# nickgreenquist/cu2rec

Measured on AMD Instinct MI355X. Metric: ratings/sec (SGD updates/sec), higher is better.
Workload: dtype f32

## Files before the change

cu2rec_amd/csrc/blocksolve.hip:

```cpp
#include <hip/hip_runtime.h>
#include <hip/hip_ext.h>

#include <algorithm>
#include <atomic>
#include <cmath>
#include <cstdlib>
#include <limits>
#include <mutex>
#include <string>
#include <utility>
#include <vector>

#include "blocksolve.hpp"
#include "blocksolve_device.hpp"
#include "blocksolve_gram.hpp"
#include "blocksolve_lookahead.hpp"
#include "blocksolve_solve.hpp"
#include "blocksolve_update.hpp"
#include "hip_check.hpp"

namespace cu2rec {

namespace {

using namespace bs_dev;

__global__ void bs_tables_kernel(SgdHyper h, float *__restrict__ t) {
    const int k = threadIdx.x;
    if (k > 2 * kB) return;
    const double a = 1.0 - static_cast<double>(h.lr) * static_cast<double>(h.q_reg);
    const double c = 1.0 - static_cast<double>(h.lr) * static_cast<double>(h.ib_reg);
    double ak = 1.0, ck = 1.0;
    for (int i = 0; i < k; ++i) {
        ak *= a;
        ck *= c;
    }
    t[kTabAdel + k] = static_cast<float>(1.0 - ak);
    t[kTabCdel + k] = static_cast<float>(1.0 - ck);
    t[kTabApow + k] = static_cast<float>(ak);
    t[kTabCpow + k] = static_cast<float>(ck);
}

__device__ __forceinline__ int lower_bound_key(const uint32_t *__restrict__ keys, int n, uint32_t target) {
    int lo = 0, hi = n;
    while (lo < hi) {
        const int mid = (lo + hi) >> 1;
        if (keys[mid] < target) lo = mid + 1; else hi = mid;
    }
    return lo;
}

__global__ __launch_bounds__(256) void bs_plan_kernel(const uint32_t *__restrict__ keys, int n_active, int n_hot,
                                                      int item_bits, int max_blocks, const int *__restrict__ item_of_rank,
                                                      int *__restrict__ chain_begin, BsChainDesc *__restrict__ chains,
                                                      BsBlockDesc *__restrict__ blocks, int *__restrict__ walk_begin, size_t stride) {
    __shared__ int s_part[256];
    const int b = blockIdx.x, tid = threadIdx.x;
    const uint32_t *kb = keys + static_cast<size_t>(b) * stride;
    int *cb = chain_begin + static_cast<size_t>(b) * (n_hot + 1);
    BsChainDesc *cd = chains + static_cast<size_t>(b) * max(n_hot, 1);
    BsBlockDesc *bd = blocks + static_cast<size_t>(b) * max_blocks;
    for (int r = tid; r <= n_hot; r += 256) cb[r] = lower_bound_key(kb, n_active, static_cast<uint32_t>(r));
    __syncthreads();
    if (tid == 0) walk_begin[b] = cb[n_hot];
    const int per = (n_hot + 255) / 256;
    const int r0 = min(tid * per, n_hot), r1 = min(r0 + per, n_hot);
    int mine = 0;
    for (int r = r0; r < r1; ++r) mine += (cb[r + 1] - cb[r] + kB - 1) / kB;
    s_part[tid] = mine;
    __syncthreads();
    __shared__ int s_total;
    if (tid == 0) {
        int run = 0;
        for (int t = 0; t < 256; ++t) {
            const int v = s_part[t];
            s_part[t] = run;
            run += v;
        }
        s_total = run;
    }
    __syncthreads();
    int off = s_part[tid];
    for (int r = r0; r < r1; ++r) {
        const int begin = cb[r], len = cb[r + 1] - begin;
        cd[r] = BsChainDesc{begin, len, off, item_of_rank[r]};
        const int nb = (len + kB - 1) / kB;
        for (int m = 0; m < nb; ++m) bd[off + m] = BsBlockDesc{begin + kB * m, min(kB, len - kB * m), r, m};
        off += nb;
    }
    for (int g = s_total + tid; g < max_blocks; g += 256) bd[g] = BsBlockDesc{0, 0, 0, 0};
}

__global__ __launch_bounds__(256, 4) void bs_gram_kernel(SgdArgs a, BsIteration it) {
    extern __shared__ float4 bs_smem[];
    const int g = static_cast<int>(blockIdx.x) - it.la_grid;
    __builtin_amdgcn_s_setprio(2);
    struct Through {
        unsigned long long *count;
        __device__ ~Through() {
            if (count && threadIdx.x == 0)
                __hip_atomic_fetch_add(count + 16 * (blockIdx.x & 31), 1ull, __ATOMIC_RELAXED, __HIP_MEMORY_SCOPE_AGENT);
        }
    } through_count{it.gram_done};
    if (g < 0) {
        const BsChainDesc last = it.chains[it.la_ranks - 1];
        const int la_end = min(last.blk0 + (last.len + kB - 1) / kB, it.la_cap);
        for (int gb = g + it.la_grid; gb < la_end; gb += it.la_grid) gram_cross_block(a, it, gb, bs_smem);
        return;
    }
    gram_block(a, it, g, bs_smem);
}

template <int SW>
__global__ __launch_bounds__(512) void bs_solve_kernel(SgdArgs a, BsIteration it) {
    extern __shared__ float4 bs_smem[];
    if (it.gram_done && threadIdx.x == 0)
        __hip_atomic_fetch_add(it.solve_started, 1ull, __ATOMIC_RELAXED, __HIP_MEMORY_SCOPE_AGENT);
    const int chain = blockIdx.x;
    const BsChainDesc cd = it.chains[chain];
    if constexpr (SW <= 8) {
        if (chain_is_lookahead(it, chain, cd)) {
            chain_lookahead<(4 * SW < kLaMaxSlots ? 4 * SW : kLaMaxSlots)>(a, it, bs_smem, cd);
            return;
        }
    }
    solve_chain<SW>(a, it, bs_smem, cd);
}

__global__ __launch_bounds__(64 * kUpdMaxWaves) void bs_update_kernel(SgdArgs a, BsIteration it) {
    const int g = blockIdx.x;
    __builtin_amdgcn_s_setprio(2);
    if (g == it.launch_blocks) {
        if (threadIdx.x == 0) await_iteration_end(it);
        return;
    }
    for (int blk = g; blk < it.max_blocks; blk += it.launch_blocks) {
        if (it.blocks[blk].n_valid == 0) break;
        update_block(a, it, blk);
    }
}

template <int SW>
void launch_solve_sw(const SgdArgs &a, const BsIteration &it, hipStream_t stream) {
    size_t lds = solve_lds_bytes(a.nslots, SW);
    if (it.la_ranks > 0) lds = std::max(lds, la_lds_bytes(a.nslots));
    ensure_max_dynamic_lds(reinterpret_cast<const void *>(bs_solve_kernel<SW>));
    hipLaunchKernelGGL((bs_solve_kernel<SW>), dim3(it.n_hot), dim3(512), lds, stream, a, it);
    const hipError_t err = hipGetLastError();
    if (err != hipSuccess)
        fail(CU2REC_EHIP, std::string("bs_solve_kernel launch failed: ") + hipGetErrorString(err) + " (SW " + std::to_string(SW) +
                              ", chains " + std::to_string(it.n_hot) + ", LDS " + std::to_string(lds) + " bytes)");
}

}

namespace {
__global__ void bs_probe_wait_kernel(const unsigned *word, unsigned *result, unsigned long long ticks) {
    if (threadIdx.x != 0) return;
    const unsigned long long t0 = wall_clock64();
    unsigned seen = 0;
    for (;;) {
        if (ld_agent(word) != 0u) {
            seen = 1;
            break;
        }
        __builtin_amdgcn_s_sleep(8);
        if (wall_clock64() - t0 > ticks) break;
    }
    __hip_atomic_store(result, seen ? 1u : 2u, __ATOMIC_RELAXED, __HIP_MEMORY_SCOPE_AGENT);
}

__global__ void bs_probe_signal_kernel(unsigned *word) {
    if (threadIdx.x == 0) __hip_atomic_store(word, 1u, __ATOMIC_RELAXED, __HIP_MEMORY_SCOPE_AGENT);
}

bool probe_streams(hipStream_t waiter, hipStream_t signaller, unsigned *scratch) {
    CU2REC_HIP(hipMemsetAsync(scratch, 0, 64 * sizeof(unsigned), waiter));
    CU2REC_HIP(hipStreamSynchronize(waiter));
    CU2REC_HIP(hipStreamSynchronize(signaller));
    hipLaunchKernelGGL(bs_probe_wait_kernel, dim3(1), dim3(64), 0, waiter, scratch, scratch + 32, 1000000ull);
    hipLaunchKernelGGL(bs_probe_signal_kernel, dim3(1), dim3(64), 0, signaller, scratch);
    CU2REC_HIP(hipGetLastError());
    CU2REC_HIP(hipStreamSynchronize(waiter));
    CU2REC_HIP(hipStreamSynchronize(signaller));
    unsigned result = 0;
    CU2REC_HIP(hipMemcpy(&result, scratch + 32, sizeof(unsigned), hipMemcpyDeviceToHost));
    return result == 1u;
}

int topology(DeviceRuntime &r, hipStream_t stream, hipStream_t side) {
    if (r.topology >= 0) return r.topology;
    if (const char *env = std::getenv("CU2REC_BS_GATE")) {
        r.topology = std::atoi(env) != 0 ? DeviceRuntime::kTopologyDevice : DeviceRuntime::kTopologyEvents;
        r.topology_forced = true;
        r.topology_why = std::string("CU2REC_BS_GATE=") + env;
        return r.topology;
    }
    if (const char *pmc = std::getenv("ROCPROF_COUNTER_COLLECTION"))
        if (*pmc && std::string(pmc) != "0" && std::string(pmc) != "False" && std::string(pmc) != "false") {
            r.topology = DeviceRuntime::kTopologyEvents;
            r.topology_why = "a rocprofv3 counter pass (ROCPROF_COUNTER_COLLECTION) serialises kernels across streams";
            return r.topology;
        }
    const bool forward = probe_streams(stream, side, r.probe);
    const bool backward = forward && probe_streams(side, stream, r.probe);
    if (forward && backward) {
        r.topology = DeviceRuntime::kTopologyDevice;
        r.topology_why = "two-stream handshake probe passed in both directions";
    } else {
        r.topology = DeviceRuntime::kTopologyEvents;
        r.topology_why = std::string("two-stream handshake probe: a wait kernel on the ") + (forward ? "side" : "main") +
                         " stream was not reached by the other stream's signal kernel within 10 ms (the streams do not run side by side here)";
    }
    return r.topology;
}

unsigned long long wait_ticks() {
    static const unsigned long long ticks = [] {
        double sec = 2.0;
        if (const char *env = std::getenv("CU2REC_BS_WAIT_S")) sec = std::max(0.001, std::atof(env));
        return static_cast<unsigned long long>(sec * 1e8);
    }();
    return ticks;
}

#ifdef CU2REC_TEST_HOOKS
int dbg() {
    static const int bits = std::getenv("CU2REC_BS_DBG") ? std::atoi(std::getenv("CU2REC_BS_DBG")) : 0;
    return bits;
}
#else
constexpr int dbg() { return 0; }
#endif

__global__ void bs_gate_kernel(const unsigned long long *count, unsigned long long target, const unsigned long long *started,
                               unsigned long long started_target, unsigned long long wait_ticks) {
    const int lane = threadIdx.x;
    const unsigned long long t0 = wall_clock64();
    unsigned polls = 0;
    for (;;) {
        unsigned long long v = lane < 32 ? ld_agent(count + 16 * lane) : 0ull;
#pragma unroll
        for (int off = 16; off > 0; off >>= 1) v += __shfl_xor(v, off);
        const unsigned long long sum = __shfl(v, 0);
        const unsigned long long st = ld_agent(started);
        if (sum >= target && st >= started_target) break;
        __builtin_amdgcn_s_sleep(16);
        if ((++polls & 63u) == 0 && wall_clock64() - t0 > wait_ticks) break;
    }
}

__global__ void bs_signal_kernel(unsigned long long *word, unsigned long long value) {
    if (threadIdx.x == 0) __hip_atomic_store(word, value, __ATOMIC_RELAXED, __HIP_MEMORY_SCOPE_AGENT);
}

void launch_gram(const SgdArgs &a, const BsIteration &it, hipStream_t stream, hipEvent_t stop) {
    const size_t gram_lds = gram_lds_bytes(a.nslots, it.la_ranks > 0);
    ensure_max_dynamic_lds(reinterpret_cast<const void *>(bs_gram_kernel));
    const int grid = it.max_blocks + (it.la_ranks > 0 ? it.la_grid : 0);
    if (stop) hipExtLaunchKernelGGL(bs_gram_kernel, dim3(grid), dim3(256), static_cast<uint32_t>(gram_lds), stream, nullptr, stop, 0, a, it);
    else hipLaunchKernelGGL(bs_gram_kernel, dim3(grid), dim3(256), gram_lds, stream, a, it);
    CU2REC_HIP(hipGetLastError());
}

void launch_solve(const SgdArgs &a, const BsIteration &it, hipStream_t stream) {
    const int sw = (a.nslots + 3) / 4;
    if (sw <= 1) launch_solve_sw<1>(a, it, stream);
    else if (sw <= 2) launch_solve_sw<2>(a, it, stream);
    else if (sw <= 4) launch_solve_sw<4>(a, it, stream);
    else if (sw <= 7) launch_solve_sw<7>(a, it, stream);
    else if (sw <= 8) launch_solve_sw<8>(a, it, stream);
    else if (sw <= 12) launch_solve_sw<12>(a, it, stream);
    else if (sw <= 16) launch_solve_sw<16>(a, it, stream);
    else fail(CU2REC_EUNSUPPORTED, "block-solve mode is compiled for n_factors <= 252");
}

void launch_update(const SgdArgs &a, const BsIteration &it, hipStream_t stream) {
    const int nwaves = (4 * a.nslots + 63) / 64;
    hipLaunchKernelGGL(bs_update_kernel, dim3(it.launch_blocks + (it.side_seq ? 1 : 0)), dim3(64 * nwaves), 0, stream, a, it);
    CU2REC_HIP(hipGetLastError());
}

std::atomic<int> g_lookahead{-1};
std::atomic<float> g_min_rate{-2.f};
constexpr float kDefaultRate = 240.f;

float min_rate_state() {
    float cur = g_min_rate.load();
    if (cur == -2.f) {
        float init = -1.f;
        if (const char *env = std::getenv("CU2REC_BLOCKSOLVE_RATE")) init = std::max(0.01f, static_cast<float>(std::atof(env)));
        g_min_rate.compare_exchange_strong(cur, init);
        cur = g_min_rate.load();
    }
    return cur;
}
}

int blocksolve_lookahead_blocks(int blocks) {
    int prev = g_lookahead.load();
    if (prev < 0) {
        const char *env = std::getenv("CU2REC_BLOCKSOLVE_LOOKAHEAD");
        const int init = env ? std::max(0, std::atoi(env)) : 24;
        g_lookahead.compare_exchange_strong(prev, init);
        prev = g_lookahead.load();
    }
    if (blocks >= 0) g_lookahead.store(blocks);
    return prev;
}

float blocksolve_min_rate(float rate) {
    const float prev = min_rate_state();
    if (rate > 0.f) g_min_rate.store(rate);
    else if (rate < 0.f) g_min_rate.store(-1.f);
    return prev > 0.f ? prev : -1.f;
}

int blocksolve_hot_items(const std::vector<double> &rate, int n_active, int rank_limit) {
    const float state = min_rate_state();
    float min_rate = state > 0.f ? state : kDefaultRate;
    const int n_cols = static_cast<int>(rate.size());
    if (state <= 0.f) {
        min_rate = std::max(30.f, min_rate * static_cast<float>(n_active) / 131072.f);
        if (n_cols > 0 && n_active <= 131072 / 4 && rate[0] < 350.0) min_rate = rate[0] >= 150.0 ? 60.f : std::numeric_limits<float>::infinity();
    }
    int n = 0;
    while (n < n_cols && rate[n] >= min_rate) ++n;
    return std::min(n, rank_limit);
}

BlockSolve::BlockSolve(int n_hot_, const std::vector<double> &rate, double hot_rate, int n_active_, int item_bits_, int max_batch_,
                       const int *item_of_rank_)
    : n_hot(n_hot_), n_active(n_active_), item_bits(item_bits_), max_batch(max_batch_), item_of_rank(item_of_rank_) {
    max_blocks = n_active / kBsLinks + n_hot + 1;
    const double bound = (hot_rate + 8.0 * std::sqrt(hot_rate) + 64.0) / kBsLinks + n_hot + 1;
    launch_blocks = std::max(1, bound >= static_cast<double>(max_blocks) ? max_blocks : static_cast<int>(bound));
    if (dbg() & 512) launch_blocks = std::min(3, max_blocks);
    const int la_min = blocksolve_lookahead_blocks(-1);
    double la_blocks = 0.0;
    while (la_min > 0 && la_ranks < n_hot && rate[la_ranks] >= static_cast<double>(la_min) * kBsLinks) {
        la_blocks += std::ceil(rate[la_ranks] / kBsLinks) + 1.0;
        ++la_ranks;
    }
    if (la_ranks > 0) la_cap = std::min(max_blocks, static_cast<int>(la_blocks * 1.25) + 4 * la_ranks + 8);
    for (int slot = 0; slot < 2; ++slot) {
        chain_begin[slot].allocate(static_cast<size_t>(max_batch) * (n_hot + 1));
        walk_begin[slot].allocate(max_batch);
        chains[slot].allocate(static_cast<size_t>(max_batch) * n_hot);
        blocks[slot].allocate(static_cast<size_t>(max_batch) * max_blocks);
    }
    tables.allocate(kBsTableFloats);
    Mbuf.allocate(static_cast<size_t>(max_blocks) * kBsRecFloats);
    ebuf.allocate(static_cast<size_t>(max_blocks) * kBsLinks);
    solve_started.allocate(16);
    solve_started.zero();
    gram_done.allocate(32 * 16);
    gram_done.zero();
    side_seq.allocate(16);
    side_seq.zero();
    if (la_cap > 0) Nbuf.allocate(static_cast<size_t>(la_cap) * kBsCrossFloats);
}

BlockSolve::~BlockSolve() {
    if (upd) (void)hipStreamDestroy(upd);
    for (hipEvent_t e : {ev_call, ev_upd, ev_gram})
        if (e) (void)hipEventDestroy(e);
}

void BlockSolve::plan(int slot, const uint32_t *sk, int nb, size_t stride, hipStream_t sched) {
    hipLaunchKernelGGL(bs_plan_kernel, dim3(nb), dim3(256), 0, sched, sk, n_active, n_hot, item_bits, max_blocks, item_of_rank,
                       chain_begin[slot].ptr, chains[slot].ptr, blocks[slot].ptr, walk_begin[slot].ptr, stride);
}

void BlockSolve::begin(const SgdArgs &a, hipStream_t stream) {
    if (a.nslots < 1 || a.nslots > kBsMaxSlots) fail(CU2REC_EUNSUPPORTED, "block-solve mode is compiled for n_factors <= 252");
    const bool same = tables_valid && tables_for.lr == a.h.lr && tables_for.q_reg == a.h.q_reg && tables_for.ib_reg == a.h.ib_reg;
    if (!same) {
        hipLaunchKernelGGL(bs_tables_kernel, dim3(1), dim3(192), 0, stream, a.h, tables.ptr);
        tables_for = a.h;
        tables_valid = true;
    }
    if (qstart_ld != a.ldq) {
        CU2REC_HIP(hipStreamSynchronize(stream));
        qstart.allocate(static_cast<size_t>(max_blocks) * a.ldq);
        qstart_ld = a.ldq;
    }
    if (!upd) {
        CU2REC_HIP(hipStreamCreateWithFlags(&upd, hipStreamNonBlocking));
        for (hipEvent_t *e : {&ev_call, &ev_upd, &ev_gram}) CU2REC_HIP(hipEventCreateWithFlags(e, hipEventDisableTiming));
    }
    unsigned *status = nullptr;
    {
        std::lock_guard<std::mutex> lock(device_runtime_mutex());
        DeviceRuntime &r = device_runtime();
        device_join = topology(r, stream, upd) == DeviceRuntime::kTopologyDevice;
        status = r.status + DeviceRuntime::kBlocksolveWord;
        host_status = r.host_status + 1;
    }
    CU2REC_HIP(hipEventRecord(ev_call, stream));
    CU2REC_HIP(hipStreamWaitEvent(upd, ev_call, 0));
    const bool la_on = la_ranks > 0 && la_supported(a.nslots);
    it = BsIteration{};
    it.n_active = n_active;
    it.n_hot = n_hot;
    it.item_mask = (1u << item_bits) - 1u;
    it.item_of_rank = item_of_rank;
    it.tables = tables.ptr;
    it.log2a = static_cast<float>(std::log2(1.0 - static_cast<double>(a.h.lr) * static_cast<double>(a.h.q_reg)));
    it.log2c = static_cast<float>(std::log2(1.0 - static_cast<double>(a.h.lr) * static_cast<double>(a.h.ib_reg)));
    it.Mbuf = Mbuf.ptr;
    it.ebuf = ebuf.ptr;
    it.qstart = qstart.ptr;
    it.max_blocks = max_blocks;
    it.launch_blocks = launch_blocks;
    it.la_ranks = la_on ? la_ranks : 0;
    it.la_cap = la_cap;
    it.la_grid = la_on ? la_cap : 0;
    it.Nbuf = Nbuf.ptr;
    it.status = status;
    it.solve_started = solve_started.ptr;
    it.wait_ticks = wait_ticks();
    if (device_join) {
        it.gram_done = gram_done.ptr;
        it.side_seq = side_seq.ptr;
    }
    upd_pending = false;
}

void BlockSolve::iteration(const SgdArgs &a, int slot, int b, const uint32_t *keys, const uint64_t *vals, bool last, hipStream_t stream,
                           const SideChains &side) {
    it.keys = keys;
    it.vals = vals;
    it.chains = chains[slot].ptr + static_cast<size_t>(b) * n_hot;
    it.blocks = blocks[slot].ptr + static_cast<size_t>(b) * max_blocks;
    it.walk_begin = walk_begin[slot].ptr + b;
    it.side_target = device_join ? side_seq_host + 1 : 0;
    if (upd_pending) CU2REC_HIP(hipStreamWaitEvent(stream, ev_upd, 0));
    launch_gram(a, it, stream, device_join ? nullptr : ev_gram);
    if (device_join) gram_done_target += static_cast<unsigned long long>(max_blocks + it.la_grid);
    else CU2REC_HIP(hipStreamWaitEvent(upd, ev_gram, 0));
    launch_solve(a, it, stream);
    if (device_join) {
        started_total += static_cast<unsigned long long>(n_hot);
        hipLaunchKernelGGL(bs_gate_kernel, dim3(1), dim3(64), 0, upd, gram_done.ptr, gram_done_target + ((dbg() & 32) ? (1ull << 40) : 0ull),
                           solve_started.ptr, started_total, it.wait_ticks);
        CU2REC_HIP(hipGetLastError());
    }
    side(upd, !device_join || last ? ev_upd : nullptr);
    if (device_join) {
        ++side_seq_host;
        if (!(dbg() & 16)) {
            hipLaunchKernelGGL(bs_signal_kernel, dim3(1), dim3(64), 0, upd, side_seq.ptr, side_seq_host);
            CU2REC_HIP(hipGetLastError());
        }
    }
    launch_update(a, it, stream);
    upd_pending = !device_join;
}

void BlockSolve::join(hipStream_t stream) {
    CU2REC_HIP(hipStreamWaitEvent(stream, ev_upd, 0));
    upd_pending = false;
}

void BlockSolve::end(hipStream_t stream) {
    CU2REC_HIP(hipMemcpyAsync(host_status, it.status, sizeof(unsigned), hipMemcpyDeviceToHost, stream));
}

}
```

cu2rec_amd/csrc/blocksolve.hpp:

```cpp
#pragma once

#include <functional>
#include <vector>

#include <hip/hip_runtime.h>

#include <cstddef>
#include <cstdint>

#include "hip_check.hpp"
#include "kernels.hpp"

namespace cu2rec {

constexpr int kBsLinks = 64;
constexpr int kBsTableStride = 2 * kBsLinks + 1;
constexpr int kBsTableFloats = 4 * kBsTableStride;
constexpr int kBsFactorFloats = 3 * 32 * 32;
constexpr int kBsRecFloats = kBsFactorFloats + kBsLinks;
constexpr int kBsCrossFloats = kBsLinks * kBsLinks;
constexpr int kBsMaxSlots = 63;

struct BsBlockDesc {
    int pos0;
    int n_valid;
    int chain;
    int m;
};

struct BsChainDesc {
    int begin, len;
    int blk0;
    int item;
};

struct BsIteration {
    const uint32_t *keys;
    const uint64_t *vals;
    int n_active;
    int n_hot;
    uint32_t item_mask;
    const BsChainDesc *chains;
    const BsBlockDesc *blocks;
    const int *walk_begin;
    const int *item_of_rank;
    const float *tables;
    float log2a, log2c;
    float *Mbuf;
    float *ebuf;
    float *qstart;
    int max_blocks;
    int launch_blocks;
    int la_ranks;
    int la_cap;
    int la_grid;
    float *Nbuf;
    unsigned *status;
    unsigned long long *solve_started;
    const unsigned long long *side_seq;
    unsigned long long side_target;
    unsigned long long *gram_done;
    unsigned long long wait_ticks;
};

float blocksolve_min_rate(float rate);
int blocksolve_lookahead_blocks(int blocks);
int blocksolve_hot_items(const std::vector<double> &rate, int n_active, int rank_limit);

class BlockSolve {
public:
    BlockSolve(int n_hot, const std::vector<double> &rate, double hot_rate, int n_active, int item_bits, int max_batch,
               const int *item_of_rank);
    ~BlockSolve();
    BlockSolve(const BlockSolve &) = delete;
    BlockSolve &operator=(const BlockSolve &) = delete;
    void plan(int slot, const uint32_t *sk, int nb, size_t stride, hipStream_t sched);
    void begin(const SgdArgs &a, hipStream_t stream);
    using SideChains = std::function<void(hipStream_t side, hipEvent_t stop)>;
    void iteration(const SgdArgs &a, int slot, int b, const uint32_t *keys, const uint64_t *vals, bool last, hipStream_t stream,
                   const SideChains &side);
    void join(hipStream_t stream);
    void end(hipStream_t stream);

    const int n_hot;

private:
    int n_active, item_bits, max_batch;
    const int *item_of_rank;
    int max_blocks;
    int launch_blocks;
    int la_ranks = 0;
    int la_cap = 0;
    DeviceBuffer<int> chain_begin[2], walk_begin[2];
    DeviceBuffer<BsChainDesc> chains[2];
    DeviceBuffer<BsBlockDesc> blocks[2];
    DeviceBuffer<float> tables, Mbuf, ebuf, qstart, Nbuf;
    int qstart_ld = 0;
    SgdHyper tables_for{};
    bool tables_valid = false;
    DeviceBuffer<unsigned long long> solve_started, gram_done, side_seq;
    unsigned long long gram_done_target = 0, started_total = 0, side_seq_host = 0;
    hipStream_t upd = nullptr;
    hipEvent_t ev_call = nullptr, ev_upd = nullptr, ev_gram = nullptr;
    BsIteration it{};
    bool device_join = false;
    bool upd_pending = false;
    unsigned *host_status = nullptr;
};

}
```

cu2rec_amd/csrc/blocksolve_gram.hpp:

```cpp
#pragma once

#include "blocksolve_device.hpp"
#include "mfma_f32.hpp"

namespace cu2rec {
namespace bs_dev {

constexpr int kGramTabFloats = 2 * kB;
__host__ __device__ inline size_t gram_tile_float4s(int nslots) { return static_cast<size_t>(kB) * (nslots | 1); }

__host__ __device__ inline int gram_tab_offset(int RS) { return max(4 * kB * RS, 5 * kH * kMS); }
__host__ __device__ inline size_t gram_lds_bytes(int nslots, bool with_cross_blocks) {
    const size_t own = static_cast<size_t>(gram_tab_offset(nslots | 1) + kGramTabFloats + kB) * sizeof(float);
    const size_t cross = with_cross_blocks ? 2 * gram_tile_float4s(nslots) * sizeof(float4) : 0;
    return own > cross ? own : cross;
}

__device__ __forceinline__ void gram_block(const SgdArgs &a, const BsIteration &it, int g, float4 *bs_smem) {
    const int wave = threadIdx.x >> 6, lane = threadIdx.x & 63;
    const BsBlockDesc bd = it.blocks[g];
    if (bd.n_valid == 0) return;
    const int nslots = a.nslots, RS = nslots | 1;
    float4 *tile = bs_smem;
    float *Ms = reinterpret_cast<float *>(bs_smem);
    float *Ns = Ms + 2 * kH * kMS;
    float *tab = Ms + gram_tab_offset(RS);
    float *basev = tab + kGramTabFloats;
    const bool mine = lane < bd.n_valid;
    const uint64_t val = it.vals[bd.pos0 + min(lane, bd.n_valid - 1)];
    const int x = static_cast<int>(val >> 32);
    if (wave == 3) {
        const float r0 = (__uint_as_float(static_cast<uint32_t>(val)) - a.global_bias) - a.user_bias[x];
        basev[lane] = mine ? r0 : 0.f;
        tab[lane] = it.tables[kTabApow + lane];
        tab[kB + lane] = it.tables[kTabCpow + lane];
    }
    const int rsub = lane >> 3, cs = lane & 7;
    const int nch = (nslots + 7) >> 3;
    for (int c0 = 0; c0 < nch; c0 += 4) {
        float4 v[2][4];
#pragma unroll
        for (int pp = 0; pp < 2; ++pp) {
            const int xr = __shfl(x, 16 * wave + 8 * pp + rsub);
            const float4 *src = reinterpret_cast<const float4 *>(a.P + static_cast<size_t>(xr) * a.ldp);
#pragma unroll
            for (int c = 0; c < 4; ++c) v[pp][c] = src[min(8 * (c0 + c) + cs, nslots - 1)];
        }
#pragma unroll
        for (int pp = 0; pp < 2; ++pp) {
            const int row = 16 * wave + 8 * pp + rsub;
#pragma unroll
            for (int c = 0; c < 4; ++c) {
                const int slot = 8 * (c0 + c) + cs;
                if (slot < nslots) tile[row * RS + slot] = row < bd.n_valid ? v[pp][c] : zero4();
            }
        }
    }
    __syncthreads();
    const int k = lane & 31, h = lane >> 5;
    f32x16 acc;
#pragma unroll
    for (int i = 0; i < 16; ++i) acc[i] = 0.f;
    if (wave < 3) {
        const int S0 = (nslots + 1) >> 1;
        const float4 *ra = tile + (wave == 1 ? kH + k : k) * RS, *rb = tile + (wave == 0 ? k : kH + k) * RS;
        for (int c = 0; c < S0; c += 2) {
            float4 va[2], vb[2];
#pragma unroll
            for (int i = 0; i < 2; ++i) {
                const int slot = h * S0 + c + i;
                const bool ok = c + i < S0 && slot < nslots;
                const float4 t0 = ra[min(slot, nslots - 1)], t1 = rb[min(slot, nslots - 1)];
                va[i] = ok ? t0 : zero4();
                vb[i] = ok ? t1 : zero4();
            }
#pragma unroll
            for (int i = 0; i < 2; ++i) {
                const float pa[4] = {va[i].x, va[i].y, va[i].z, va[i].w}, pb[4] = {vb[i].x, vb[i].y, vb[i].z, vb[i].w};
#pragma unroll
                for (int e = 0; e < 4; ++e) acc = __builtin_amdgcn_mfma_f32_32x32x2f32(pa[e], pb[e], acc, 0, 0, 0);
            }
        }
    }
    __syncthreads();
    if (wave < 3) {
        const float lr = a.h.lr;
        const int K = (wave == 0 ? 0 : kH) + k;
        const int J0 = (wave == 1 ? kH : 0) + 4 * h;
        const bool row_ok = K < bd.n_valid;
        float *dst = Ns + (wave * kH + k) * kMS + 4 * h;
#pragma unroll
        for (int m = 0; m < 4; ++m) {
            f32x4 out;
#pragma unroll
            for (int e = 0; e < 4; ++e) {
                const int d = K - 1 - (J0 + 8 * m + e);
                const float fd = static_cast<float>(d);
                const float v = lr * (__builtin_amdgcn_exp2f(fd * it.log2c) + __builtin_amdgcn_exp2f(fd * it.log2a) * acc[4 * m + e]);
                out[e] = d >= 0 && row_ok ? v : 0.f;
            }
            *reinterpret_cast<f32x4 *>(dst + 8 * m) = out;
        }
    }
    __syncthreads();
    if (wave == 0) {
    float m[kH];
    {
        const float *Nh = Ns + h * kH * kMS;
        float4 cur[8], nxt[8];
        m[0] = k == 0 ? 1.f : 0.f;
        cur[0] = *reinterpret_cast<const float4 *>(Nh + kMS);
#pragma unroll
        for (int kk = 1; kk < kH; ++kk) {
            if (kk + 1 < kH) {
#pragma unroll
                for (int i4 = 0; i4 < (kk + 4) / 4; ++i4) nxt[i4] = *reinterpret_cast<const float4 *>(Nh + (kk + 1) * kMS + 4 * i4);
            }
            __builtin_amdgcn_sched_barrier(0);
            float s[4] = {kk == k ? 1.f : 0.f, 0.f, 0.f, 0.f};
#pragma unroll
            for (int i4 = 0; i4 < (kk + 3) / 4; ++i4) {
                const float nv[4] = {cur[i4].x, cur[i4].y, cur[i4].z, cur[i4].w};
#pragma unroll
                for (int e = 0; e < 4; ++e)
                    if (4 * i4 + e < kk) s[e] = __builtin_fmaf(-nv[e], m[4 * i4 + e], s[e]);
            }
            m[kk] = (s[0] + s[1]) + (s[2] + s[3]);
            __builtin_amdgcn_sched_barrier(0);
            if (kk + 1 < kH) {
#pragma unroll
                for (int i4 = 0; i4 < (kk + 4) / 4; ++i4) cur[i4] = nxt[i4];
            }
        }
    }
#pragma unroll
    for (int kk = 0; kk < kH; ++kk) Ms[(h * kH + kk) * kMS + k] = m[kk];
    __builtin_amdgcn_wave_barrier();
    f32x16 tacc, macc;
#pragma unroll
    for (int i = 0; i < 16; ++i) tacc[i] = macc[i] = 0.f;
    {
        const float4 *arow = reinterpret_cast<const float4 *>(Ns + (2 * kH + k) * kMS + 16 * h);
#pragma unroll
        for (int t4 = 0; t4 < 4; ++t4) {
            const float4 a4 = arow[t4];
            const float av[4] = {a4.x, a4.y, a4.z, a4.w};
#pragma unroll
            for (int e = 0; e < 4; ++e)
                tacc = __builtin_amdgcn_mfma_f32_32x32x2f32(av[e], Ms[(16 * h + 4 * t4 + e) * kMS + k], tacc, 0, 0, 0);
        }
        const float *mrow = Ms + (kH + k) * kMS + 4 * h;
#pragma unroll
        for (int t4 = 0; t4 < 4; ++t4) {
            const float4 a4 = *reinterpret_cast<const float4 *>(mrow + 8 * t4);
            const float av[4] = {a4.x, a4.y, a4.z, a4.w};
#pragma unroll
            for (int e = 0; e < 4; ++e) macc = __builtin_amdgcn_mfma_f32_32x32x2f32(av[e], tacc[4 * t4 + e], macc, 0, 0, 0);
        }
    }
#pragma unroll
    for (int reg = 0; reg < 16; ++reg) Ns[acc_row(reg, h) * kMS + k] = -macc[reg];
    }
    __syncthreads();
    float *rec = it.Mbuf + static_cast<size_t>(g) * kBsRecFloats;
    {
        const int t = threadIdx.x, row = t >> 3, c4 = t & 7;
        const float *src[3] = {Ms, Ns, Ms + kH * kMS};
#pragma unroll
        for (int q = 0; q < 3; ++q) *reinterpret_cast<f32x4 *>(rec + q * kH * kH + 4 * t) = *reinterpret_cast<const f32x4 *>(src[q] + row * kMS + 4 * c4);
        if (t < kB / 4) *reinterpret_cast<f32x4 *>(rec + kBsFactorFloats + 4 * t) = *reinterpret_cast<const f32x4 *>(basev + 4 * t);
    }
}

__device__ __forceinline__ void gram_cross_block(const SgdArgs &a, const BsIteration &it, int g, float4 *smem) {
    const BsBlockDesc bd = it.blocks[g];
    if (bd.n_valid == 0 || bd.m == 0 || !chain_is_lookahead(it, bd.chain, it.chains[bd.chain])) return;
    const int wave = threadIdx.x >> 6, lane = threadIdx.x & 63, k = lane & 31, h = lane >> 5;
    const int rt = wave >> 1, ct = wave & 1;
    const int nslots = a.nslots, RS = nslots | 1, S0 = (nslots + 1) >> 1;
    float4 *tile_c = smem, *tile_p = smem + kB * RS;
    {
        const int xc = static_cast<int>(it.vals[bd.pos0 + min(lane, bd.n_valid - 1)] >> 32);
        const int xp = static_cast<int>(it.vals[bd.pos0 - kB + lane] >> 32);
        const int rsub = lane >> 3, cs = lane & 7;
        const int nch = (nslots + 7) >> 3;
        for (int c0 = 0; c0 < nch; c0 += 2) {
            float4 vc[2][2], vp[2][2];
#pragma unroll
            for (int pp = 0; pp < 2; ++pp) {
                const int src_lane = 16 * wave + 8 * pp + rsub;
                const float4 *sc = reinterpret_cast<const float4 *>(a.P + static_cast<size_t>(__shfl(xc, src_lane)) * a.ldp);
                const float4 *sp = reinterpret_cast<const float4 *>(a.P + static_cast<size_t>(__shfl(xp, src_lane)) * a.ldp);
#pragma unroll
                for (int c = 0; c < 2; ++c) {
                    vc[pp][c] = sc[min(8 * (c0 + c) + cs, nslots - 1)];
                    vp[pp][c] = sp[min(8 * (c0 + c) + cs, nslots - 1)];
                }
            }
#pragma unroll
            for (int pp = 0; pp < 2; ++pp) {
                const int row = 16 * wave + 8 * pp + rsub;
#pragma unroll
                for (int c = 0; c < 2; ++c) {
                    const int slot = 8 * (c0 + c) + cs;
                    if (slot < nslots) {
                        tile_c[row * RS + slot] = row < bd.n_valid ? vc[pp][c] : zero4();
                        tile_p[row * RS + slot] = vp[pp][c];
                    }
                }
            }
        }
    }
    __syncthreads();
    f32x16 acc;
#pragma unroll
    for (int i = 0; i < 16; ++i) acc[i] = 0.f;
    {
        const float4 *ra = tile_c + (kH * rt + k) * RS, *rb = tile_p + (kH * ct + k) * RS;
        for (int c = 0; c < S0; c += 2) {
            float4 va[2], vb[2];
#pragma unroll
            for (int i = 0; i < 2; ++i) {
                const int slot = h * S0 + c + i;
                const bool ok = c + i < S0 && slot < nslots;
                const float4 t0 = ra[min(slot, nslots - 1)], t1 = rb[min(slot, nslots - 1)];
                va[i] = ok ? t0 : zero4();
                vb[i] = ok ? t1 : zero4();
            }
#pragma unroll
            for (int i = 0; i < 2; ++i) {
                const float pa[4] = {va[i].x, va[i].y, va[i].z, va[i].w}, pb[4] = {vb[i].x, vb[i].y, vb[i].z, vb[i].w};
#pragma unroll
                for (int e = 0; e < 4; ++e) acc = __builtin_amdgcn_mfma_f32_32x32x2f32(pa[e], pb[e], acc, 0, 0, 0);
            }
        }
    }
    const float lr = a.h.lr;
    float *dst = it.Nbuf + static_cast<size_t>(g) * kBsCrossFloats;
    const int j = kH * ct + k;
#pragma unroll
    for (int reg = 0; reg < 16; ++reg) {
        const int i = kH * rt + acc_row(reg, h);
        const float fd = static_cast<float>(kB - 1 + i - j);
        const float v = lr * (__builtin_amdgcn_exp2f(fd * it.log2c) + __builtin_amdgcn_exp2f(fd * it.log2a) * acc[reg]);
        dst[i * kB + j] = i < bd.n_valid ? v : 0.f;
    }
    __syncthreads();
}

}
}
```

Before: 1.769 billion.

## Launch gram kernel over launch_blocks and loop blocks persistently

The gram kernel grid shrinks from max_blocks to launch_blocks (gram_blocks), and each workgroup walks its blocks with a stride of gram_blocks until it reaches an empty descriptor. The next block descriptor is prefetched, and the block fields are forced to be wave-uniform with readfirstlane. This avoids launching many empty workgroups when max_blocks is a loose upper bound. In exchange, blocks beyond the first are processed serially within a workgroup, with a barrier between them, and the device-join counter target is adjusted to match the new grid size.

```diff
diff --git a/cu2rec_amd/csrc/blocksolve.hip b/cu2rec_amd/csrc/blocksolve.hip
--- a/cu2rec_amd/csrc/blocksolve.hip
+++ b/cu2rec_amd/csrc/blocksolve.hip
@@ -108,7 +108,22 @@
         for (int gb = g + it.la_grid; gb < la_end; gb += it.la_grid) gram_cross_block(a, it, gb, bs_smem);
         return;
     }
-    gram_block(a, it, g, bs_smem);
+    BsBlockDesc bd = it.blocks[g];
+    asm volatile("" : "+v"(bd.pos0), "+v"(bd.n_valid));
+    bd.pos0 = __builtin_amdgcn_readfirstlane(bd.pos0);
+    bd.n_valid = __builtin_amdgcn_readfirstlane(bd.n_valid);
+    for (int blk = g; bd.n_valid != 0;) {
+        const int nxt = blk + it.gram_blocks;
+        const BsBlockDesc nbd = it.blocks[min(nxt, it.max_blocks - 1)];
+        int tidx = threadIdx.x;
+        asm volatile("" : "+v"(tidx));
+        gram_block(a, it, blk, bd, tidx, bs_smem);
+        if (nxt >= it.max_blocks || nbd.n_valid == 0) break;
+        __syncthreads();
+        bd.pos0 = __builtin_amdgcn_readfirstlane(nbd.pos0);
+        bd.n_valid = __builtin_amdgcn_readfirstlane(nbd.n_valid);
+        blk = nxt;
+    }
 }
 
 template <int SW>
@@ -257,7 +272,7 @@
 void launch_gram(const SgdArgs &a, const BsIteration &it, hipStream_t stream, hipEvent_t stop) {
     const size_t gram_lds = gram_lds_bytes(a.nslots, it.la_ranks > 0);
     ensure_max_dynamic_lds(reinterpret_cast<const void *>(bs_gram_kernel));
-    const int grid = it.max_blocks + (it.la_ranks > 0 ? it.la_grid : 0);
+    const int grid = it.gram_blocks + (it.la_ranks > 0 ? it.la_grid : 0);
     if (stop) hipExtLaunchKernelGGL(bs_gram_kernel, dim3(grid), dim3(256), static_cast<uint32_t>(gram_lds), stream, nullptr, stop, 0, a, it);
     else hipLaunchKernelGGL(bs_gram_kernel, dim3(grid), dim3(256), gram_lds, stream, a, it);
     CU2REC_HIP(hipGetLastError());
@@ -336,6 +351,7 @@
     const double bound = (hot_rate + 8.0 * std::sqrt(hot_rate) + 64.0) / kBsLinks + n_hot + 1;
     launch_blocks = std::max(1, bound >= static_cast<double>(max_blocks) ? max_blocks : static_cast<int>(bound));
     if (dbg() & 512) launch_blocks = std::min(3, max_blocks);
+    gram_blocks = (dbg() & 1024) ? std::min(2, max_blocks) : launch_blocks;
     const int la_min = blocksolve_lookahead_blocks(-1);
     double la_blocks = 0.0;
     while (la_min > 0 && la_ranks < n_hot && rate[la_ranks] >= static_cast<double>(la_min) * kBsLinks) {
@@ -413,6 +429,7 @@
     it.qstart = qstart.ptr;
     it.max_blocks = max_blocks;
     it.launch_blocks = launch_blocks;
+    it.gram_blocks = gram_blocks;
     it.la_ranks = la_on ? la_ranks : 0;
     it.la_cap = la_cap;
     it.la_grid = la_on ? la_cap : 0;
@@ -437,7 +454,7 @@
     it.side_target = device_join ? side_seq_host + 1 : 0;
     if (upd_pending) CU2REC_HIP(hipStreamWaitEvent(stream, ev_upd, 0));
     launch_gram(a, it, stream, device_join ? nullptr : ev_gram);
-    if (device_join) gram_done_target += static_cast<unsigned long long>(max_blocks + it.la_grid);
+    if (device_join) gram_done_target += static_cast<unsigned long long>(it.gram_blocks + it.la_grid);
     else CU2REC_HIP(hipStreamWaitEvent(upd, ev_gram, 0));
     launch_solve(a, it, stream);
     if (device_join) {
diff --git a/cu2rec_amd/csrc/blocksolve.hpp b/cu2rec_amd/csrc/blocksolve.hpp
--- a/cu2rec_amd/csrc/blocksolve.hpp
+++ b/cu2rec_amd/csrc/blocksolve.hpp
@@ -51,6 +51,7 @@
     float *qstart;
     int max_blocks;
     int launch_blocks;
+    int gram_blocks;
     int la_ranks;
     int la_cap;
     int la_grid;
@@ -89,6 +90,7 @@
     const int *item_of_rank;
     int max_blocks;
     int launch_blocks;
+    int gram_blocks;
     int la_ranks = 0;
     int la_cap = 0;
     DeviceBuffer<int> chain_begin[2], walk_begin[2];
diff --git a/cu2rec_amd/csrc/blocksolve_gram.hpp b/cu2rec_amd/csrc/blocksolve_gram.hpp
--- a/cu2rec_amd/csrc/blocksolve_gram.hpp
+++ b/cu2rec_amd/csrc/blocksolve_gram.hpp
@@ -16,10 +16,8 @@
     return own > cross ? own : cross;
 }
 
-__device__ __forceinline__ void gram_block(const SgdArgs &a, const BsIteration &it, int g, float4 *bs_smem) {
-    const int wave = threadIdx.x >> 6, lane = threadIdx.x & 63;
-    const BsBlockDesc bd = it.blocks[g];
-    if (bd.n_valid == 0) return;
+__device__ __forceinline__ void gram_block(const SgdArgs &a, const BsIteration &it, int g, const BsBlockDesc &bd, int tidx, float4 *bs_smem) {
+    const int wave = __builtin_amdgcn_readfirstlane(tidx >> 6), lane = tidx & 63;
     const int nslots = a.nslots, RS = nslots | 1;
     float4 *tile = bs_smem;
     float *Ms = reinterpret_cast<float *>(bs_smem);
@@ -164,7 +162,7 @@
     __syncthreads();
     float *rec = it.Mbuf + static_cast<size_t>(g) * kBsRecFloats;
     {
-        const int t = threadIdx.x, row = t >> 3, c4 = t & 7;
+        const int t = tidx, row = t >> 3, c4 = t & 7;
         const float *src[3] = {Ms, Ns, Ms + kH * kMS};
 #pragma unroll
         for (int q = 0; q < 3; ++q) *reinterpret_cast<f32x4 *>(rec + q * kH * kH + 4 * t) = *reinterpret_cast<const f32x4 *>(src[q] + row * kMS + 4 * c4);
```

New measurement: 1.782 billion (median of 6 runs). No clear change (+0.8%).
